# HeadReaper-hc/PL-inertial-slam

Measured on AMD Instinct MI355X. Metric: local-BA iterations/sec (50 KF, 20k pts, 4k lines, IMU), higher is better.
Workload: dtype f64; 1 GPU; configs[2]: 50 KF / 20k points / 4k lines + IMU preintegration edges (9-DoF PVR + 6-DoF bias vertices); K=50, points=20000, lines=4000, point_obs=86023, line_obs=17197, pose_dim=735, dense_dim=357, banded_twisted_solve=False, twin_factorisation=True, fused_landmark_passes=True

## Files before the change

### include/plba.h

```cpp
#ifndef PLBA_H
#define PLBA_H

#include <stddef.h>
#include <stdint.h>

#ifdef __cplusplus
extern "C" {
#endif

typedef struct plba_problem plba_problem;

typedef enum {
    PLBA_OK = 0,
    PLBA_ERR_INVALID = -1,
    PLBA_ERR_STATE = -2,
    PLBA_ERR_DEVICE = -3,
    PLBA_ERR_NUMERIC = -4,
    PLBA_ERR_EXCHANGE = -5
} plba_status;

typedef enum {
    PLBA_EDGE_POINT = 0,
    PLBA_EDGE_LINE = 1,
    PLBA_EDGE_IMU_PVR = 2,
// ... 12 lines not shown
    int    device;
    int    use_mfma;
    int    profile;
    int    factor_block;
    int    factor_flow;
    int    chain_elim;
    int    wide_steps;
    int    band_solve;
    int    marg_exact;
    int    lm_fused;
    int    lm_fused_min_obs;
    int    lm_group_steps;
    int    chain_seg;
    int    twin_max_tiles;
    int    diag;
    int    pgo_solver;
} plba_options;
#define PLBA_DIAG_TIMING 1
#define PLBA_DIAG_MARG_DUMP 2
#define PLBA_DIAG_LEAD_WAIT_FAIL 4
#define PLBA_DIAG_NO_MARG_PREROTATE 8

void plba_default_options(plba_options* o);

typedef struct {
    int    iterations;
    int    trials;
    int    stop_reason;
    int    solver_failures;
    double chi2_initial;
// ... 289 lines not shown
```

### pl-inertial-slam_amd/abi.py

```python
import ctypes as C
import numpy as np

c_double_p = C.POINTER(C.c_double)
c_int32_p = C.POINTER(C.c_int32)
c_uint8_p = C.POINTER(C.c_uint8)

EDGE_POINT, EDGE_LINE, EDGE_IMU_PVR, EDGE_IMU_BIAS, EDGE_PRIOR = range(5)

STATUS = {0: "PLBA_OK", -1: "PLBA_ERR_INVALID", -2: "PLBA_ERR_STATE", -3: "PLBA_ERR_DEVICE",
          -4: "PLBA_ERR_NUMERIC", -5: "PLBA_ERR_EXCHANGE"}


class Options(C.Structure):
    _fields_ = [("tau", C.c_double), ("good_step_lower", C.c_double), ("good_step_upper", C.c_double),
                ("max_trials", C.c_int), ("user_lambda_init", C.c_double), ("marg_eps", C.c_double),
                ("fix_line_position_jacobian", C.c_int),
                ("device", C.c_int), ("use_mfma", C.c_int), ("profile", C.c_int), ("factor_block", C.c_int), ("factor_flow", C.c_int), ("chain_elim", C.c_int), ("wide_steps", C.c_int), ("band_solve", C.c_int), ("marg_exact", C.c_int), ("lm_fused", C.c_int),
                ("lm_fused_min_obs", C.c_int), ("lm_group_steps", C.c_int), ("chain_seg", C.c_int), ("twin_max_tiles", C.c_int), ("diag", C.c_int),
                ("pgo_solver", C.c_int)]


class Stats(C.Structure):
    _fields_ = [("iterations", C.c_int), ("trials", C.c_int), ("stop_reason", C.c_int),
                ("solver_failures", C.c_int), ("chi2_initial", C.c_double), ("chi2_final", C.c_double),
                ("lambda_final", C.c_double), ("ms_total", C.c_double), ("ms_phase", C.c_double * 8)]


class TraceRow(C.Structure):
    _fields_ = [("iteration", C.c_int), ("trial", C.c_int), ("accepted", C.c_int), ("solver_ok", C.c_int),
                ("lam", C.c_double), ("chi2_current", C.c_double), ("chi2_trial", C.c_double),
                ("scale", C.c_double), ("rho", C.c_double)]


class Prior(C.Structure):
# ... 839 lines not shown
```

### pl-inertial-slam_amd/csrc/plba_api.hip

```cpp
#include <atomic>
#include <algorithm>
#include <thread>
#include <array>
#include <chrono>
#include <cmath>
#include <cstdio>
#include <cstring>
#include <condition_variable>
#include <functional>
#include <map>
#include <mutex>

#include "plba_problem.h"

using namespace plba;

namespace {
char g_create_err[256] = "";
static std::mutex g_ctx_mu;
static std::vector<HostCtx> g_ctx_free;
static std::map<int, hipStream_t> g_lib_stream;
static std::vector<plba_problem*> g_parked;
static const size_t PARK_MAX = 2;
}
// ... 45 lines not shown
    o->good_step_lower = 1. / 3.;
    o->good_step_upper = 2. / 3.;
    o->max_trials = 10;
    o->user_lambda_init = 0.0;
    o->marg_eps = 1e-8;
    o->device = -1;
    o->use_mfma = 1;
    o->factor_block = 32;
    o->factor_flow = 0;
    o->chain_elim = 1;
    o->wide_steps = 0;
    o->band_solve = 1;
    o->marg_exact = 1;
    o->lm_fused = 1;
    o->lm_fused_min_obs = 40000;
}
const char* plba_backend_name(void) { return "hip-gfx950"; }
const char* plba_last_error(const plba_problem* p) { return p ? p->err : g_create_err; }

int plba_create(const plba_options* opt, plba_problem** out) {
    if (!out) { snprintf(g_create_err, sizeof g_create_err, "out is NULL"); return PLBA_ERR_INVALID; }
    *out = nullptr;
    int ndev = 0;
    hipError_t e = hipGetDeviceCount(&ndev);
    if (e != hipSuccess || ndev == 0) {
        snprintf(g_create_err, sizeof g_create_err, "no HIP device available (%s); the plba product path has no CPU fallback",
                 e == hipSuccess ? "0 devices" : hipGetErrorString(e));
        return PLBA_ERR_DEVICE;
    }
    {
// ... 957 lines not shown
    d.imu_i = p->d_imu_i.p; d.imu_j = p->d_imu_j.p; d.imu_pre = p->d_imu_pre.p; d.imu_info_pvr = p->d_imu_ipvr.p; d.imu_info_bias = p->d_imu_ibias.p;
    d.imu_err = p->d_imu_err.p; d.imu_chi = p->d_imu_chi.p;
    d.pr_n = p->pr_n; d.pr_nv = p->pr_nv;
    d.pr_kf = p->d_pr_kf.p; d.pr_isbias = p->d_pr_isbias.p; d.pr_size = p->d_pr_size.p; d.pr_idx = p->d_pr_idx.p;
    d.pr_x0off = p->d_pr_x0off.p; d.pr_off = p->d_pr_off.p; d.pr_x0 = p->d_pr_x0.p; d.pr_J0 = p->d_pr_J0.p; d.pr_r0 = p->d_pr_r0.p;
    if (pr_dev) { d.pr_x0 = pr_dev; d.pr_J0 = pr_dev + pr_nx; d.pr_r0 = pr_dev + pr_nx + (size_t)p->pr_n * p->pr_n; }
    d.pr_err = p->d_pr_err.p; d.pr_dx = p->d_pr_dx.p; d.pr_chi = p->d_pr_chi.p;
    d.Hconst = p->d_Hconst.p; d.Himu = p->d_Himu.p; d.bimu = p->d_bimu.p; d.Himu_alt = p->d_Himu2.p; d.bimu_alt = p->d_bimu2.p; d.bprior = p->d_bprior.p; d.bprior_alt = p->d_bprior2.p; d.sys = p->d_sys.p; d.Lfac = p->d_Lfac.p; d.bpg = p->d_bpg.p; d.x = p->d_x.p;
    d.Linv = p->d_Linv.p; d.flow_flags = p->d_flow_flags.p; d.LTblk = p->d_LT32.p; d.Linv32 = p->d_LT32.p; d.rdblk = p->d_rd32.p; d.fb = (p->opt.factor_block == 64) ? 64 : 32; d.chol_flags = p->d_chol_flags.p; d.flow = p->opt.factor_flow != 0; d.wide = p->opt.wide_steps != 0 && !d.flow;
    d.chi_part = p->d_chi_part.p; d.scale_part = p->d_scale_part.p; d.maxd_part = p->d_maxd_part.p; d.kfdiag = p->d_kfdiag.p; d.posediag = p->d_posediag.p;
    d.ctrl = p->d_ctrl.p; d.trace = p->d_trace.p; d.trace_cap = TRACE_CAP; d.trace_n = p->d_trace_n.p;
    std::vector<int32_t> skey;
    {
        skey.reserve(64 + 2 * (size_t)K + 2 * (size_t)M + 4 * (size_t)p->pr_nv + ((size_t)K * K + 3) / 4 * 2 + K);
        for (int v : {K, M, p->pr_nv, p->pr_n, (int)lm_cand, p->world, p->rank, p->opt.chain_elim, p->opt.use_mfma, p->opt.factor_block, p->opt.factor_flow, p->opt.wide_steps, p->opt.band_solve,
                      p->opt.chain_seg, p->opt.twin_max_tiles, (int)(E > 300000), (int)p->lm_disable, p->P}) skey.push_back(v);
        skey.insert(skey.end(), p->off_pvr.begin(), p->off_pvr.end()); skey.insert(skey.end(), p->off_bias.begin(), p->off_bias.end());
        skey.insert(skey.end(), w.imu_i.begin(), w.imu_i.end()); skey.insert(skey.end(), w.imu_j.begin(), w.imu_j.end());
        skey.insert(skey.end(), pr_kf.begin(), pr_kf.end()); skey.insert(skey.end(), pr_isb.begin(), pr_isb.end()); skey.insert(skey.end(), p->pr_size.begin(), p->pr_size.begin() + p->pr_nv); skey.insert(skey.end(), pr_off.begin(), pr_off.end());
        skey.insert(skey.end(), p->pr_idx.begin(), p->pr_idx.begin() + p->pr_nv);
        auto pack = [&](const std::vector<uint8_t>& v) { for (size_t i = 0; i < v.size(); i += 4) { int32_t w = 0; for (size_t j = i; j < std::min(i + 4, v.size()); ++j) w |= (int32_t)(v[j] & 0xFF) << (8 * (j - i)); skey.push_back(w); } };
        pack(cov);
        if (lm_cand) { pack(LH.cov); skey.insert(skey.end(), LH.row_kf.begin(), LH.row_kf.end()); skey.push_back(LH.wmax); }
    }
    const bool sc_hit = p->sc.valid && skey == p->sc.key;
    struct BatchSwitch {
        DevBatch* prev; std::vector<std::pair<void*, size_t>>* prevlog;
        BatchSwitch(DevBatch* b, std::vector<std::pair<void*, size_t>>* log) : prev(darr_batch()), prevlog(darr_zero_log()) { darr_batch() = b; darr_zero_log() = log; }
        ~BatchSwitch() { darr_batch() = prev; darr_zero_log() = prevlog; }
    };
    if (sc_hit) {
// ... 193 lines not shown
                            }
                        for (int idx = 0; idx < n * 9; ++idx) oR[idx] = cidx[(size_t)i0 * 9 + idx] >= 0 ? cidx[(size_t)i0 * 9 + idx] : -1;
                    }
                    if ((size_t)p->Ppad * ld >= ((size_t)1 << 30)) ok = false;
                    HIPCK(p, p->d_esrc.upload(esrc));
                    cv.esrc = p->d_esrc.p; cv.esrc_off = nullptr;
                }
                p->d_W.release();
                HIPCK(p, p->d_W.alloc((size_t)(nel * 9 + 4) * cv.Wld)); HIPCK(p, p->d_Ldinv.alloc((size_t)nel * 81)); HIPCK(p, p->d_Lsub.alloc((size_t)nel * 81));
                const size_t sysn_d = (size_t)(cv.Pdpad + TILE) * cv.Pdpad;
                HIPCK(p, p->d_sysd.alloc(sysn_d)); HIPCK(p, p->d_Lfacd.alloc(sysn_d)); HIPCK(p, p->d_xd.alloc(cv.Pdpad));
                HIPCK(p, p->d_Linvd.alloc((size_t)((cv.Pdpad + TILE - 1) / TILE) * TILE * TILE)); HIPCK(p, p->d_LT32d.alloc((size_t)cv.Pdpad * 64)); HIPCK(p, p->d_rd32d.alloc(cv.Pdpad));
                HIPCK(p, p->d_flow_flagsd.alloc((cv.Pdpad + TILE - 1) / TILE)); HIPCK(p, p->d_chol_flagsd.alloc((size_t)(cv.Pdpad / 32 + 2) * (cv.Pdpad / 32)));
                cv.cidx = p->d_cidx.p; cv.epos = p->d_epos.p; cv.seg_start = p->d_seg_start.p; cv.seg_col = p->d_seg_col.p;
                cv.pidx = p->d_pidx.p; cv.ppos = p->d_ppos.p; cv.pslot = p->d_pslot.p; cv.slotcol = p->d_slotcol.p;
                cv.W = p->d_W.p; cv.Ldinv = p->d_Ldinv.p; cv.Lsub = p->d_Lsub.p;
                DevBuf& dd = p->dd;
                dd = d;
                dd.P = cv.Pd; dd.Ppad = cv.Pdpad; dd.ld = cv.Pdpad;
                dd.sys = p->d_sysd.p; dd.Lfac = p->d_Lfacd.p; dd.x = p->d_xd.p; dd.Linv = p->d_Linvd.p; dd.LTblk = p->d_LT32d.p; dd.Linv32 = p->d_LT32d.p;
                dd.rdblk = p->d_rd32d.p; dd.flow_flags = p->d_flow_flagsd.p; dd.chol_flags = p->d_chol_flagsd.p;
                dd.Ninv = nullptr; dd.Nwork = nullptr;
                if (cv.Pdpad / 32 <= NINV_MAX_T) { HIPCK(p, p->d_Ninvd.alloc((size_t)2 * cv.Pdpad * cv.Pdpad)); dd.Ninv = p->d_Ninvd.p; dd.Nwork = dd.Ninv + (size_t)cv.Pdpad * cv.Pdpad; }
                p->chain_ok = true;
            }
        }
    }
    lap("chain maps + buffers");
    d.Ninv = nullptr; d.Nwork = nullptr;
    HIPCK(p, p->d_dbgbuf.alloc(128)); d.dbgbuf = p->d_dbgbuf.p; p->dd.dbgbuf = d.dbgbuf;
    if (!p->chain_ok && p->P > 0 && p->Ppad / 32 <= NINV_MAX_T) { HIPCK(p, p->d_Ninv.alloc((size_t)2 * p->Ppad * p->ld)); d.Ninv = p->d_Ninv.p; d.Nwork = d.Ninv + (size_t)p->Ppad * p->ld; }
// ... 167 lines not shown
        }
        for (int r = 0; r < p->Ppad; ++r) xl.push_back(r * ld + r);
        std::sort(xl.begin(), xl.end());
        xl.erase(std::unique(xl.begin(), xl.end()), xl.end());
        HIPCK(p, p->d_xlist.upload(xl));
        d.xlist = p->d_xlist.p; d.nxlist = (int)xl.size();
    }
    p->band_ok = false; p->twin_ok = false;
    for (double& v : p->plan_twin) v = 0.0;
    p->dd.band = 0; p->dd.twin_m0 = 0; p->dd.twin_fac = nullptr; p->dd.cs_order = nullptr; p->dd.perm = nullptr; p->dd.xmap = nullptr; p->dd.alt = nullptr; p->dd.alt2 = nullptr;
    p->dd.wtw = nullptr;
    if (p->chain_ok && p->lm_ok && p->world <= 1) {
        const int T = p->cv.Pdpad / 32;
        HIPCK(p, p->d_wtw.alloc((size_t)(T * (T + 1) / 2 + T) * 1024, false));
        p->dd.wtw = p->d_wtw.p;
    }
    int plan_hbt = -1;
    if (p->chain_ok && p->opt.band_solve && !p->dv.flow && !p->dv.wide) {
        const ChainView& cv = p->cv;
        const int T = cv.Pdpad / 32;
        int hbt = 0;
        if (T >= 8) {
            const std::vector<int32_t>& hpidx = p->h_pidx; const std::vector<int32_t>& hsegcol = p->h_seg_col;
            std::vector<int32_t> dense_of(p->ld, -1);
            for (int c = 0; c < cv.Pd; ++c) dense_of[hpidx[c]] = c;
            for (int32_t idx : p->h_alist) {
                const int r = dense_of[idx / p->ld], c = dense_of[idx % p->ld];
                if (r >= 0 && c >= 0) hbt = std::max(hbt, std::abs(r / 32 - c / 32));
            }
            for (int g = 0; g < cv.nseg; ++g) if (hsegcol[2 * g + 1] > hsegcol[2 * g]) hbt = std::max(hbt, (hsegcol[2 * g + 1] - 1) / 32 - hsegcol[2 * g] / 32);
// ... 992 lines not shown
        std::vector<double> h; HIPCK(p, fetch(d.erec, ((size_t)p->win.Ep + 2 * (size_t)p->win.El) * EREC_UNIT, h));
        if (w == "err_pt") { v.resize((size_t)p->win.Ep * 2); for (int e = 0; e < p->win.Ep; ++e) { const size_t o = (size_t)p->ob_pos[e] * EREC_UNIT; v[2 * (size_t)e] = h[o + EREC_PT_E0]; v[2 * (size_t)e + 1] = h[o + EREC_PT_E0 + 1]; } }
        else { v.assign((size_t)p->win.El * 3, 0.0); for (int e = 0; e < p->win.El; ++e) { const size_t o = (size_t)p->ob_pos[p->win.Ep + e] * EREC_UNIT; v[3 * (size_t)e] = h[o + 13]; v[3 * (size_t)e + 1] = h[o + 14]; } }
    } else if (w == "erec") {
        if (p->lm_ok) FAIL(p, PLBA_ERR_STATE, "\"erec\": the fused landmark passes keep no record table");
        HIPCK(p, fetch(d.erec, ((size_t)p->win.Ep + 2 * (size_t)p->win.El) * EREC_UNIT, v));
    }
    else if (w == "stamps") { HIPCK(p, fetch(d.maxd_part, 80, v)); }
    else if (w == "dbgbuf") { HIPCK(p, fetch(d.dbgbuf, 128, v)); }
    else if (w == "pose_dim") v = {(double)p->P};
    else if (w == "marg_path") v.assign(p->marg_path, p->marg_path + 5);
    else if (w == "prof_lin_launches") v = {(double)p->prof_lin_launches};
    else if (w == "lm_groups") v = p->lm_hist;
    else if (w == "lm_fused") v = {(double)(p->lm_ok ? 1 : 0), (double)p->lv.ngrp, (double)p->lv.nblk, p->lm_ok && p->lm_hist.size() > 18 ? p->lm_hist[18] : 0.0 };
    else if (w == "marg_J") v = p->marg_dbg;
    else if (w == "dense_dim") v = {(double)(p->chain_ok ? p->cv.Pd : p->P)};
    else if (w == "band") v = {(double)(p->band_ok ? 1 : 0)};
    else if (w == "twin") v = {(double)(p->twin_ok ? 1 : 0)};
    else if (w == "solver_plan") {
        const bool ninv = !p->band_ok && (p->chain_ok ? p->dd.Ninv : p->dv.Ninv) != nullptr;
        v = {(double)(p->band_ok ? 3 : p->twin_ok ? 2 : p->chain_ok ? 1 : 0), (double)((p->chain_ok ? p->cv.Pdpad : p->Ppad) / 32), ninv ? 1.0 : 0.0, (double)p->plan_hbt,
             p->plan_twin[0], p->plan_twin[1], p->plan_twin[2], p->plan_twin[3], p->plan_twin[4], (double)(p->band_ok ? p->bandv.nA : 0), (double)(p->band_ok ? p->bandv.nB : 0)};
    }
    else if (w == "fact_launches_estimate") v = {(double)p->seg_launch_est};
    else if (w == "fact_launches") {
        if (p->band_ok) v = {2.0};
        else if (p->twin_ok) v = {(double)(p->twinv.nlaunch + (p->twinv.T - p->twinv.final0 - 1))};
        else v = {-1.0};
    }
    else if (w == "chi2") { HIPCK(p, plba_d2h(p, p->h_ctrl, d.ctrl, sizeof(Ctrl))); v = {p->h_ctrl->current_chi}; }
// ... 10 lines not shown
```

### pl-inertial-slam_amd/csrc/plba_chain.hip

```cpp
#include "plba_internal.h"
#include "plba_chain_dev.h"
#include "plba_factor32_dev.h"

namespace plba {

__global__ __launch_bounds__(ELIM_THREADS) void k_chain_elim(DevBuf d, ChainView cv) {
    __shared__ __attribute__((aligned(16))) ChainElimLds LDS;
    chain_elim_segment(d, cv, blockIdx.x, LDS);
}

template <bool PRE>
__global__ __launch_bounds__(256) void k_chain_schur(DevBuf d, ChainView cv, DevBuf dd) {
    __shared__ __attribute__((aligned(16))) double sC0[32 * LS];
    __shared__ __attribute__((aligned(16))) Look32 S0;
    const int T = cv.Pdpad / 32;
    const int b = blockIdx.x;
    int ta, tb;
    chain_schur_tile_of(cv, dd, b, ta, tb);
    const int wv = threadIdx.x >> 6, lane = threadIdx.x & 63, li = lane & 15, lk = lane >> 4;
    const int tr = wv >> 1, tc = wv & 1;
    const int ldd = dd.ld;
    const bool rhs_row = (ta == T);
    double4v acc;
    if (PRE) acc = *reinterpret_cast<const double4v*>(dd.wtw + (size_t)b * 1024 + 4 * threadIdx.x);
    double aold[4];
    {
        const int cb = tb * 32 + tc * 16 + li;
        const int pb = cb < cv.Pd ? cv.pidx[cb] : 0;
#pragma unroll
        for (int v = 0; v < 4; ++v) {
            const int lr = tr * 16 + lk + 4 * v;
// ... 30 lines not shown
            if (fsel >= 0) sC0[(frev ? 31 - lr : lr) * LS + (frev ? 31 - lc : lc)] = out;
        }
    }
    if (fsel < 0 || dd.flow || dd.wide || dd.band) return;
    factor32_reset(S0, threadIdx.x);
    __syncthreads();
    factor32_tile<false>(dd, fsel & 0xffff, sC0, S0, wv, lane);
}

void launch_chain_elim(const DevBuf& d, const ChainView& cv, hipStream_t s) {
    hipLaunchKernelGGL(k_chain_elim, dim3(cv.nseg), dim3(ELIM_THREADS), 0, s, d, cv);
}
bool chain_schur_factors_tile0(const DevBuf& dd) { return !dd.flow && !dd.wide && !dd.band; }
void launch_chain_schur(const DevBuf& d, const ChainView& cv, const DevBuf& dd, hipStream_t s, bool products_done) {
    const int T = cv.Pdpad / 32;
    if (products_done) hipLaunchKernelGGL(k_chain_schur<true>, dim3(T * (T + 1) / 2 + T), dim3(256), 0, s, d, cv, dd);
    else hipLaunchKernelGGL(k_chain_schur<false>, dim3(T * (T + 1) / 2 + T), dim3(256), 0, s, d, cv, dd);
}

}
```

### pl-inertial-slam_amd/csrc/plba_chain_dev.h

```cpp
#pragma once
#include "plba_internal.h"

namespace plba {

typedef double double4v __attribute__((ext_vector_type(4)));

namespace chain_detail {
__device__ __forceinline__ double lane_bcast(double v, int l) {
    int lo = __double2loint(v), hi = __double2hiint(v);
    lo = __builtin_amdgcn_readlane(lo, l);
    hi = __builtin_amdgcn_readlane(hi, l);
    return __hiloint2double(hi, lo);
}
__device__ __forceinline__ double rsqrt_full(double d) {
    double y = __builtin_amdgcn_rsq(d);
    y = y * fma(-0.5 * d * y, y, 1.5);
    y = y * fma(-0.5 * d * y, y, 1.5);
    return y;
}
template <typename T> __device__ __forceinline__ void lds_store(T* p, T v) { __hip_atomic_store(p, v, __ATOMIC_RELAXED, __HIP_MEMORY_SCOPE_WORKGROUP); }
template <typename T> __device__ __forceinline__ T lds_load(const T* p) { return __hip_atomic_load(const_cast<T*>(p), __ATOMIC_RELAXED, __HIP_MEMORY_SCOPE_WORKGROUP); }
__device__ __forceinline__ double sym_at(const double* sys, int ld, int i, int j) { return i >= j ? sys[(size_t)i * ld + j] : sys[(size_t)j * ld + i]; }
constexpr int SPIN_MAX = 1 << 20;
constexpr int SEGMAX = CHAIN_SEG;
// ... 222 lines not shown
#pragma unroll
            for (int u = 0; u < 8; ++u) {
                const int r = s0 + 32 * ch + 4 * u + lk;
                const bool in = r < rhi;
                av[ch][u] = in ? Wa[(size_t)r * cv.Wld] : 0.0;
                bv[ch][u] = in ? Wb[(size_t)r * cv.Wld] : 0.0;
            }
#pragma unroll
        for (int ch = 0; ch < NCH; ++ch)
#pragma unroll
            for (int u = 0; u < 8; ++u) acc = __builtin_amdgcn_mfma_f64_16x16x4f64(av[ch][u], bv[ch][u], acc, 0, 0, 0);
    }
    return acc;
}

}
```

### pl-inertial-slam_amd/csrc/plba_internal.h

```cpp
#pragma once
#include <hip/hip_runtime.h>
#include <stdint.h>
#include <map>
#include <mutex>
#include <string>
#include <utility>
#include <vector>

#include "plba.h"
#include "plba_math.h"
#include "plba_twin_plan.h"

namespace plba {

constexpr int TILE = 64;

inline hipError_t ensure_dyn_lds(const void* func, int bytes) {
    static std::mutex mu;
    static std::map<std::pair<int, const void*>, int> done;
    int dev = 0;
    hipError_t e = hipGetDevice(&dev);
    if (e != hipSuccess) return e;
    std::lock_guard<std::mutex> lk(mu);
    auto it = done.find({dev, func});
// ... 173 lines not shown
    const int32_t* ppos;
    const int32_t* pslot;
    const int32_t* slotcol;
    const int32_t* trow;
    const int32_t* kfpos;
    const int32_t* ekf;
    const int32_t* ukf;
    int nukf;
    const int32_t* esrc;
    const int32_t* esrc_off;
    const int32_t* bkf;
    const int32_t* imu_loc;
    double* W;
    double* Ldinv;
    double* Lsub;
};
constexpr int BAND_HB = 3;
constexpr int TWIN_MAX_TILES = 64;
constexpr int BAND_MIN_TILES = 24;
struct BandView {
    int T, nA, nB;
    double* Lband;
    double* y;
    double* mid;
};
size_t band_lds_bytes(int Pdpad);
void launch_band_solve(const DevBuf& dd, const BandView& bv, hipStream_t s);
void launch_chain_elim(const DevBuf& d, const ChainView& cv, hipStream_t s);
void launch_chain_schur(const DevBuf& d, const ChainView& cv, const DevBuf& dd, hipStream_t s, bool products_done = false);
struct TwinView {
// ... 28 lines not shown
```

### pl-inertial-slam_amd/csrc/plba_kernels.hip

```cpp
#include "plba_internal.h"
#include "plba_chain_dev.h"

namespace plba {

#define DEV __device__ __forceinline__

DEV double wave_sum(double v) {
#pragma unroll
    for (int o = 32; o > 0; o >>= 1) v += __shfl_down(v, o, 64);
    return v;
}
DEV double wave_max(double v) {
#pragma unroll
    for (int o = 32; o > 0; o >>= 1) v = fmax(v, __shfl_down(v, o, 64));
    return v;
}
DEV double block_sum_256(double v, double* s4) {
    v = wave_sum(v);
    int w = threadIdx.x >> 6;
    if ((threadIdx.x & 63) == 0) s4[w] = v;
    __syncthreads();
    double r = 0;
    if (threadIdx.x == 0) r = (s4[0] + s4[1]) + (s4[2] + s4[3]);
    __syncthreads();
// ... 677 lines not shown
    const bool ok = d.ctrl->solver_ok != 0;
    if (ok && has_pvr) kf_oplus_pvr(s, u9, tmp);
    if (ok && has_bias) {
#pragma unroll
        for (int i = 0; i < 6; ++i) tmp[16 + i] = s[16 + i] + ub6[i];
    }
}
DEV void update_kf_vals(const DevBuf& d, int trial, int k, const double* s , const double* u9, const double* ub6, bool has_pvr, bool has_bias) {
    double tmp[KF_STRIDE];
    kf_trial_state(d, s, u9, ub6, has_pvr, has_bias, tmp);
    double* o = d.kf[trial] + (size_t)k * KF_STRIDE;
#pragma unroll
    for (int i = 0; i < KF_STRIDE; ++i) publish(o + i, tmp[i]);
}

template <bool LOCAL = false>
DEV const double* chain_back_segment(const DevBuf& d, const ChainView& cv, const double* xd, const int g, const int cur, const int trial) {
    constexpr int BACK_THREADS = LMB;
    constexpr int UFAST = 5;
    __shared__ double sv[SEGMAX * 9];
    __shared__ double sxc[SEGMAX * 9];
    __shared__ double sxw[192];
    __shared__ double sM[SEGMAX][162];
#ifdef PLBA_STAMPS_LM
    unsigned long long cts[6]; cts[0] = __builtin_readcyclecounter();
#define CSTAMP(i) cts[i] = __builtin_readcyclecounter()
#else
#define CSTAMP(i) do {} while (0)
#endif
    const int wv = threadIdx.x >> 6, lane = threadIdx.x & 63, t = threadIdx.x;
    const int i0 = cv.seg_start[g], n = cv.seg_start[g + 1] - i0;
    const int wlo = cv.seg_col[2 * g], wn = cv.seg_col[2 * g + 1] - wlo;
    const int lg = t >> 4, ll = t & 15;
    constexpr int NPASS = (SEGMAX * 9 + 15) / 16;
    double wr[NPASS][UFAST], wbv[NPASS];
#pragma unroll
    for (int q = 0; q < NPASS; ++q) {
        const int r = q * 16 + lg;
        const bool in = r < n * 9;
        const double* Wr = cv.W + (size_t)(i0 * 9 + (in ? r : 0)) * cv.Wld + wlo;
#pragma unroll
        for (int u = 0; u < UFAST; ++u) { const int c = ll + 16 * u; wr[q][u] = Wr[c < wn ? c : 0]; }
        wbv[q] = Wr[cv.Pd - wlo];
    }
    int kf_k = -1, e_blk = -1;
    const int32_t* kd = nullptr;
    if (LOCAL) {}
    else if (t < n) { e_blk = t; kd = cv.bkf + (size_t)(g * CHAIN_SEG + t) * 20; }
    else if (g == 0 && t >= 64 && t - 64 < cv.nukf && t - 64 < BACK_THREADS - 64) kd = cv.bkf + (size_t)(cv.nseg * CHAIN_SEG + (t - 64)) * 20;
    double ks[KF_STRIDE];
    int op = -1, ob = -1, pc[6] = {-1, -1, -1, -1, -1, -1}, cc[9] = {-1, -1, -1, -1, -1, -1, -1, -1, -1};
    if (kd) {
        const int4* k4 = reinterpret_cast<const int4*>(kd);
        const int4 a0 = k4[0], a1 = k4[1], a2 = k4[2], a3 = k4[3], a4 = k4[4];
        kf_k = a0.x; op = a0.y; ob = a0.z;
        pc[0] = a0.w; pc[1] = a1.x; pc[2] = a1.y; pc[3] = a1.z; pc[4] = a1.w; pc[5] = a2.x;
        cc[0] = a2.y; cc[1] = a2.z; cc[2] = a2.w; cc[3] = a3.x; cc[4] = a3.y; cc[5] = a3.z; cc[6] = a3.w; cc[7] = a4.x; cc[8] = a4.y;
        const double* sp = d.kf[cur] + (size_t)kf_k * KF_STRIDE;
#pragma unroll
        for (int i = 0; i < KF_STRIDE; ++i) ks[i] = sp[i];
    }
    for (int idx = t; idx < n * 81; idx += BACK_THREADS) {
        sM[idx / 81][idx % 81] = cv.Ldinv[(size_t)i0 * 81 + idx];
        sM[idx / 81][81 + idx % 81] = cv.Lsub[(size_t)i0 * 81 + idx];
    }
    if (!LOCAL && g == 0) for (int c = t; c < cv.Pd; c += BACK_THREADS) publish(&d.x[cv.pidx[c]], xd[c]);
    for (int c = t; c < wn; c += BACK_THREADS) sxw[c] = xd[wlo + c];
    double u9[9] = {0, 0, 0, 0, 0, 0, 0, 0, 0}, ub6[6] = {0, 0, 0, 0, 0, 0};
    if (kf_k >= 0) {
        const int ps[6] = {0, 1, 2, 6, 7, 8};
#pragma unroll
        for (int i = 0; i < 6; ++i) if (pc[i] >= 0) u9[ps[i]] = xd[pc[i]];
#pragma unroll
        for (int i = 0; i < 3; ++i) if (cc[i] >= 0) u9[3 + i] = xd[cc[i]];
#pragma unroll
        for (int i = 0; i < 6; ++i) if (cc[3 + i] >= 0) ub6[i] = xd[cc[3 + i]];
    }
    __syncthreads();
    CSTAMP(1);
#pragma unroll
    for (int q = 0; q < NPASS; ++q) {
        const int r = q * 16 + lg;
        double sacc = 0.0;
#pragma unroll
        for (int u = 0; u < UFAST; ++u) { const int c = ll + 16 * u; sacc = fma(wr[q][u], c < wn ? sxw[c] : 0.0, sacc); }
        if (wn > 16 * UFAST && r < n * 9) {
            const double* Wr = cv.W + (size_t)(i0 * 9 + r) * cv.Wld + wlo;
            for (int c = 16 * UFAST + ll; c < wn; c += 16) sacc = fma(Wr[c], sxw[c], sacc);
        }
        sacc += dpp_get<0x111, 0xf>(sacc);
        sacc += dpp_get<0x112, 0xf>(sacc);
        sacc += dpp_get<0x114, 0xf>(sacc);
        sacc += dpp_get<0x118, 0xf>(sacc);
        if (ll == 15 && r < n * 9) sv[r] = wbv[q] - sacc;
    }
    __syncthreads();
    CSTAMP(2);
    if (wv == 0) {
        const int r = lane < 9 ? lane : 8;
        double xn = 0.0;
        for (int i = n - 1; i >= 0; --i) {
            const double* Li = sM[i];
            const double* Ls = Li + 81;
            double tt = sv[i * 9 + r];
            if (i + 1 < n) {
#pragma unroll
                for (int q = 0; q < 9; ++q) tt = fma(-Ls[q * 9 + r], lane_bcast(xn, q), tt);
            }
            double xi = 0.0;
#pragma unroll
            for (int q = 0; q < 9; ++q) xi = fma(Li[q * 9 + r], lane_bcast(tt, q), xi);
            xn = xi;
            const int gi = cv.cidx[(i0 + i) * 9 + r];
            if (lane < 9) { sxc[i * 9 + r] = gi >= 0 ? xi : 0.0; if (!LOCAL && gi >= 0) publish(&d.x[gi], xi); }
        }
    }
    __syncthreads();
    CSTAMP(3);
    if (LOCAL) return sxc;
    if (kf_k >= 0) {
        if (e_blk >= 0) {
#pragma unroll
            for (int i = 0; i < 3; ++i) u9[3 + i] = sxc[e_blk * 9 + i];
#pragma unroll
            for (int i = 0; i < 6; ++i) ub6[i] = sxc[e_blk * 9 + 3 + i];
            if (op >= 0) { publish(&d.x[op], u9[0]); publish(&d.x[op + 1], u9[1]); publish(&d.x[op + 2], u9[2]); publish(&d.x[op + 6], u9[6]); publish(&d.x[op + 7], u9[7]); publish(&d.x[op + 8], u9[8]); }
        }
        update_kf_vals(d, trial, kf_k, ks, u9, ub6, op >= 0, ob >= 0);
    }
    if (g == 0) for (int u = BACK_THREADS - 64 + t; u < cv.nukf; u += BACK_THREADS) update_kf_one(d, cur, trial, cv.ukf[u]);
#ifdef PLBA_STAMPS_LM
    asm volatile("s_waitcnt vmcnt(0)" ::: "memory");
    CSTAMP(4);
    if (threadIdx.x == 0 && g < 2) { for (int q = 0; q < 5; ++q) d.dbgbuf[48 + 6 * g + q] = (double)(cts[q] - cts[0]); d.dbgbuf[48 + 6 * g + 5] = (double)(long long)__builtin_amdgcn_s_memrealtime(); }
// ... 101 lines not shown
    __shared__ double sKF[2 * KF_STRIDE];
    __shared__ double sJ[9 * 24];
    __shared__ double sOJ[9 * 24];
    __shared__ double sE[16];
    __shared__ double sT[16];
    __shared__ double sW[2];
    __shared__ int sOff[24];
    const int ki = d.imu_i[m], kj = d.imu_j[m];
    const double* si = d.kf[state] + (size_t)ki * KF_STRIDE;
    const double* sj = d.kf[state] + (size_t)kj * KF_STRIDE;
    if (loc && loc->cv->imu_loc) {
        const ChainView& cvl = *loc->cv;
        const int32_t* il = cvl.imu_loc + 4 * (size_t)m;
        const int seg = il[0];
        const double* sxc = nullptr;
        if (seg >= 0) sxc = chain_back_segment<true>(d, cvl, loc->xd, seg, loc->cur, state);
        if (lane < 2) {
            const int k = lane ? kj : ki, dsc = il[1 + lane];
            const double* s = d.kf[loc->cur] + (size_t)k * KF_STRIDE;
            double ks[KF_STRIDE], u9[9] = {0, 0, 0, 0, 0, 0, 0, 0, 0}, ub6[6] = {0, 0, 0, 0, 0, 0}, tmp[KF_STRIDE];
#pragma unroll
            for (int i = 0; i < KF_STRIDE; ++i) ks[i] = s[i];
            bool has_pvr = false, has_bias = false;
            if (dsc >= 0) {
                const int32_t* kd = cvl.bkf + (size_t)dsc * 20;
                has_pvr = kd[1] >= 0; has_bias = kd[2] >= 0;
                const int ps[6] = {0, 1, 2, 6, 7, 8};
#pragma unroll
                for (int i = 0; i < 6; ++i) if (kd[3 + i] >= 0) u9[ps[i]] = loc->xd[kd[3 + i]];
                const int e = dsc - seg * CHAIN_SEG;
                if (seg >= 0 && e >= 0 && e < CHAIN_SEG && dsc < cvl.nseg * CHAIN_SEG) {
// ... 472 lines not shown
}
template <bool JAC, bool WIDE_OK>
__global__ __launch_bounds__(LMB) void k_lm_trial(DevBuf d, LmView lv, int cur, int trial, Robust rb, ChainView cv, const double* xd, int nlead, int npose, unsigned back_target, DecideArgs da) {
    static_assert(LMB == 256, "chain_back_segment's thread layout");
    __shared__ double s4[4];
    int b = blockIdx.x;
    const int nimu_first = (nlead > 0 && npose > 0 && cv.imu_loc && gridDim.x <= 512) ? min(npose, d.M) : 0;
    if (b >= nlead && b < nlead + nimu_first) {
        const LocalStates loc{&cv, xd, cur};
        pose_edge_block<JAC, 256>(d, trial, rb, b - nlead, threadIdx.x, nullptr, 0, s4, nullptr, &loc);
        if (da.fuse) trial_arrive(d, da, lv.ngrp, s4);
        return;
    }
    if (b >= nlead + nimu_first) b -= nimu_first;
    if (b < nlead) {
        chain_back_segment(d, cv, xd, b, cur, trial);
        lead_done(d.back_cnt);
    } else if (b < nlead + lv.ngrp) {
        __shared__ LmLds S;
        const int g = b - nlead;
        if (g == 0 && nlead == 0) {
            for (int k = threadIdx.x; k < d.K; k += LMB) update_kf_one(d, cur, trial, k);
            lead_done(d.back_cnt);
        }
        const int kind = lv.grp[g].kind;
        if (kind == 0) lm_trial_group<false, false>(d, lv, g, cur, trial, rb, cv, xd, nlead != 0, S);
        else if (kind == 1) lm_trial_group<true, false>(d, lv, g, cur, trial, rb, cv, xd, nlead != 0, S);
        else if (WIDE_OK && kind == 2) lm_trial_group<false, true>(d, lv, g, cur, trial, rb, cv, xd, nlead != 0, S);
        else if (WIDE_OK) lm_trial_group<true, true>(d, lv, g, cur, trial, rb, cv, xd, nlead != 0, S);
    } else {
        const int m = b - nlead - lv.ngrp + nimu_first;
// ... 246 lines not shown
```

### pl-inertial-slam_amd/csrc/plba_problem.h

```cpp
#pragma once
#include <algorithm>
#include <chrono>
#include <cstring>
#include <map>
#include <mutex>
#include <utility>
#include <vector>

#include "plba_internal.h"
#include "plba_window.h"

namespace plba {

struct DevPool {
    static constexpr size_t POOL_CAP = (size_t)8 << 30;
    std::mutex mu;
    std::map<std::pair<int, size_t>, std::vector<void*>> free_;
    size_t cached = 0;
    size_t n_malloc = 0, n_reuse = 0;
    static size_t size_class(size_t bytes) { size_t c = 4096; while (c < bytes) c <<= 1; return c; }
    hipError_t get(size_t bytes, void** out, size_t* cls) {
        int dev = 0;
        (void)hipGetDevice(&dev);
        *cls = size_class(bytes);
// ... 199 lines not shown
    plba::DArr<char> d_batch_z, d_batch_u;
    plba::DevBatch batch;
    struct StructCache {
        bool valid = false;
        std::vector<int32_t> key;
        plba::DevBuf dd;
        const int32_t *alist = nullptr, *xlist = nullptr, *alist2 = nullptr; int nalist = 0, nxlist = 0, nalist2 = 0;
        const uint8_t* col_gather = nullptr;
        double *Ninv = nullptr, *Nwork = nullptr, *dbgbuf = nullptr;
        bool chain_ok = false;
        std::vector<std::pair<void*, size_t>> zero_log;
        long hits = 0, misses = 0;
    } sc;
    plba::DArr<char> d_sbatch_z, d_sbatch_u;
    plba::DevBatch sbatch;
    plba::DArr<double> d_wtw;
    plba::DArr<double> d_twin_alt;
    plba::Window win, win_next;
    plba::SlidePlan slide;
    int pr_n = 0, pr_nv = 0;
    std::vector<int32_t> pr_vid, pr_size, pr_idx;
    std::vector<double> pr_x0, pr_J0, pr_r0;
    plba::DArr<double> d_prd[2];
    int prd_slot = 0;
    bool prior_dev = false;
    bool prior_changed = false;
    int pr_m = 0;
    plba::MargPending* mp = nullptr;
    double pgo_sparse[8] = {0, 0, 0, 0, 0, 0, 0, 0};
    long host_waits = 0;
// ... 135 lines not shown
```

Baseline: 7812 iterations/s.

## Precompute chain back-substitution map so per-trial back-solve becomes a matvec

Adds a precomputed per-segment map G, built once in extra blocks of the chain Schur kernel, that folds the block-bidiagonal back-substitution into the W coupling matrix. The per-trial chain_back_segment then reads G instead of W, skips loading Ldinv/Lsub and the serial 9x9 triangular sweep, and publishes x directly. This moves the sequential dependency chain out of the per-LM-trial critical path and into the once-per-iteration factorization. The cost is an extra G buffer and additional work in the Schur kernel. It is enabled by default through a new option.

```diff
diff --git a/include/plba.h b/include/plba.h
--- a/include/plba.h
+++ b/include/plba.h
@@ -50,6 +50,7 @@
     int    chain_seg;
     int    twin_max_tiles;
     int    diag;
+    int    chain_back_map;
     int    pgo_solver;
 } plba_options;
 #define PLBA_DIAG_TIMING 1
diff --git a/pl-inertial-slam_amd/abi.py b/pl-inertial-slam_amd/abi.py
--- a/pl-inertial-slam_amd/abi.py
+++ b/pl-inertial-slam_amd/abi.py
@@ -17,7 +17,7 @@
                 ("fix_line_position_jacobian", C.c_int),
                 ("device", C.c_int), ("use_mfma", C.c_int), ("profile", C.c_int), ("factor_block", C.c_int), ("factor_flow", C.c_int), ("chain_elim", C.c_int), ("wide_steps", C.c_int), ("band_solve", C.c_int), ("marg_exact", C.c_int), ("lm_fused", C.c_int),
                 ("lm_fused_min_obs", C.c_int), ("lm_group_steps", C.c_int), ("chain_seg", C.c_int), ("twin_max_tiles", C.c_int), ("diag", C.c_int),
-                ("pgo_solver", C.c_int)]
+                ("chain_back_map", C.c_int), ("pgo_solver", C.c_int)]
 
 
 class Stats(C.Structure):
diff --git a/pl-inertial-slam_amd/csrc/plba_api.hip b/pl-inertial-slam_amd/csrc/plba_api.hip
--- a/pl-inertial-slam_amd/csrc/plba_api.hip
+++ b/pl-inertial-slam_amd/csrc/plba_api.hip
@@ -83,6 +83,7 @@
     o->marg_exact = 1;
     o->lm_fused = 1;
     o->lm_fused_min_obs = 40000;
+    o->chain_back_map = 1;
 }
 const char* plba_backend_name(void) { return "hip-gfx950"; }
 const char* plba_last_error(const plba_problem* p) { return p ? p->err : g_create_err; }
@@ -1070,7 +1071,7 @@
     {
         skey.reserve(64 + 2 * (size_t)K + 2 * (size_t)M + 4 * (size_t)p->pr_nv + ((size_t)K * K + 3) / 4 * 2 + K);
         for (int v : {K, M, p->pr_nv, p->pr_n, (int)lm_cand, p->world, p->rank, p->opt.chain_elim, p->opt.use_mfma, p->opt.factor_block, p->opt.factor_flow, p->opt.wide_steps, p->opt.band_solve,
-                      p->opt.chain_seg, p->opt.twin_max_tiles, (int)(E > 300000), (int)p->lm_disable, p->P}) skey.push_back(v);
+                      p->opt.chain_seg, p->opt.chain_back_map, p->opt.twin_max_tiles, (int)(E > 300000), (int)p->lm_disable, p->P}) skey.push_back(v);
         skey.insert(skey.end(), p->off_pvr.begin(), p->off_pvr.end()); skey.insert(skey.end(), p->off_bias.begin(), p->off_bias.end());
         skey.insert(skey.end(), w.imu_i.begin(), w.imu_i.end()); skey.insert(skey.end(), w.imu_j.begin(), w.imu_j.end());
         skey.insert(skey.end(), pr_kf.begin(), pr_kf.end()); skey.insert(skey.end(), pr_isb.begin(), pr_isb.end()); skey.insert(skey.end(), p->pr_size.begin(), p->pr_size.begin() + p->pr_nv); skey.insert(skey.end(), pr_off.begin(), pr_off.end());
@@ -1294,7 +1295,7 @@
                 HIPCK(p, p->d_flow_flagsd.alloc((cv.Pdpad + TILE - 1) / TILE)); HIPCK(p, p->d_chol_flagsd.alloc((size_t)(cv.Pdpad / 32 + 2) * (cv.Pdpad / 32)));
                 cv.cidx = p->d_cidx.p; cv.epos = p->d_epos.p; cv.seg_start = p->d_seg_start.p; cv.seg_col = p->d_seg_col.p;
                 cv.pidx = p->d_pidx.p; cv.ppos = p->d_ppos.p; cv.pslot = p->d_pslot.p; cv.slotcol = p->d_slotcol.p;
-                cv.W = p->d_W.p; cv.Ldinv = p->d_Ldinv.p; cv.Lsub = p->d_Lsub.p;
+                cv.W = p->d_W.p; cv.Ldinv = p->d_Ldinv.p; cv.Lsub = p->d_Lsub.p; cv.G = nullptr;
                 DevBuf& dd = p->dd;
                 dd = d;
                 dd.P = cv.Pd; dd.Ppad = cv.Pdpad; dd.ld = cv.Pdpad;
@@ -1492,6 +1493,10 @@
         const int T = p->cv.Pdpad / 32;
         HIPCK(p, p->d_wtw.alloc((size_t)(T * (T + 1) / 2 + T) * 1024, false));
         p->dd.wtw = p->d_wtw.p;
+        if (p->opt.chain_back_map) {
+            HIPCK(p, p->d_G.alloc((size_t)(p->cv.nel * 9 + 4) * p->cv.Wld, false));
+            p->cv.G = p->d_G.p;
+        }
     }
     int plan_hbt = -1;
     if (p->chain_ok && p->opt.band_solve && !p->dv.flow && !p->dv.wide) {
@@ -2514,6 +2519,7 @@
     else if (w == "lm_groups") v = p->lm_hist;
     else if (w == "lm_fused") v = {(double)(p->lm_ok ? 1 : 0), (double)p->lv.ngrp, (double)p->lv.nblk, p->lm_ok && p->lm_hist.size() > 18 ? p->lm_hist[18] : 0.0 };
     else if (w == "marg_J") v = p->marg_dbg;
+    else if (w == "chain_back_map") v = {(double)(p->opt.chain_back_map ? 1 : 0), (double)((p->chain_ok && p->cv.G) ? 1 : 0)};
     else if (w == "dense_dim") v = {(double)(p->chain_ok ? p->cv.Pd : p->P)};
     else if (w == "band") v = {(double)(p->band_ok ? 1 : 0)};
     else if (w == "twin") v = {(double)(p->twin_ok ? 1 : 0)};
diff --git a/pl-inertial-slam_amd/csrc/plba_chain.hip b/pl-inertial-slam_amd/csrc/plba_chain.hip
--- a/pl-inertial-slam_amd/csrc/plba_chain.hip
+++ b/pl-inertial-slam_amd/csrc/plba_chain.hip
@@ -15,6 +15,11 @@
     __shared__ __attribute__((aligned(16))) Look32 S0;
     const int T = cv.Pdpad / 32;
     const int b = blockIdx.x;
+    if (PRE && b >= T * (T + 1) / 2 + T) {
+        __shared__ ChainMapLds sMap;
+        chain_back_map_segment(cv, b - (T * (T + 1) / 2 + T), sMap);
+        return;
+    }
     int ta, tb;
     chain_schur_tile_of(cv, dd, b, ta, tb);
     const int wv = threadIdx.x >> 6, lane = threadIdx.x & 63, li = lane & 15, lk = lane >> 4;
@@ -75,7 +80,7 @@
 bool chain_schur_factors_tile0(const DevBuf& dd) { return !dd.flow && !dd.wide && !dd.band; }
 void launch_chain_schur(const DevBuf& d, const ChainView& cv, const DevBuf& dd, hipStream_t s, bool products_done) {
     const int T = cv.Pdpad / 32;
-    if (products_done) hipLaunchKernelGGL(k_chain_schur<true>, dim3(T * (T + 1) / 2 + T), dim3(256), 0, s, d, cv, dd);
+    if (products_done) hipLaunchKernelGGL(k_chain_schur<true>, dim3(T * (T + 1) / 2 + T + (cv.G ? cv.nseg : 0)), dim3(256), 0, s, d, cv, dd);
     else hipLaunchKernelGGL(k_chain_schur<false>, dim3(T * (T + 1) / 2 + T), dim3(256), 0, s, d, cv, dd);
 }
 
diff --git a/pl-inertial-slam_amd/csrc/plba_chain_dev.h b/pl-inertial-slam_amd/csrc/plba_chain_dev.h
--- a/pl-inertial-slam_amd/csrc/plba_chain_dev.h
+++ b/pl-inertial-slam_amd/csrc/plba_chain_dev.h
@@ -260,4 +260,65 @@
     return acc;
 }
 
-}
+struct ChainMapLds {
+    alignas(16) double sM[SEGMAX][162];
+    int live[SEGMAX * 9];
+};
+__device__ __forceinline__ void chain_back_map_segment(const ChainView& cv, const int g, ChainMapLds& S) {
+    const int i0 = cv.seg_start[g], n = cv.seg_start[g + 1] - i0;
+    const int wlo = cv.seg_col[2 * g], wn = cv.seg_col[2 * g + 1] - wlo;
+    if (n <= 0) return;
+    const int lc = threadIdx.x;
+    const bool act = lc <= wn;
+    const int col = lc == wn ? cv.Pd : wlo + (act ? lc : 0);
+    constexpr int AHEAD = 3;
+    double w[SEGMAX][9];
+    auto request = [&](int j) {
+        const double* Wc = cv.W + (size_t)((i0 + (j < n ? n - 1 - j : 0)) * 9) * cv.Wld + col;
+#pragma unroll
+        for (int r = 0; r < 9; ++r) w[j][r] = Wc[(size_t)r * cv.Wld];
+    };
+#pragma unroll
+    for (int j = 0; j < AHEAD; ++j) request(j);
+    for (int idx = threadIdx.x; idx < n * 81; idx += blockDim.x) {
+        S.sM[idx / 81][idx % 81] = cv.Ldinv[(size_t)i0 * 81 + idx];
+        S.sM[idx / 81][81 + idx % 81] = cv.Lsub[(size_t)i0 * 81 + idx];
+    }
+    for (int idx = threadIdx.x; idx < n * 9; idx += blockDim.x) S.live[idx] = cv.cidx[(size_t)i0 * 9 + idx] >= 0;
+    __syncthreads();
+    if ((int)(threadIdx.x & ~63u) > wn) return;
+    double gn[9];
+#pragma unroll
+    for (int r = 0; r < 9; ++r) gn[r] = 0.0;
+#pragma unroll
+    for (int j = 0; j < SEGMAX; ++j) {
+        if (j >= n) break;
+        if (j + AHEAD < SEGMAX) request(j + AHEAD);
+        const int i = n - 1 - j;
+        const double* Li = S.sM[i];
+        const double* Ls = Li + 81;
+        double t[9];
+#pragma unroll
+        for (int r = 0; r < 9; ++r) t[r] = w[j][r];
+        if (j > 0) {
+#pragma unroll
+            for (int q = 0; q < 9; ++q)
+#pragma unroll
+                for (int r = 0; r < 9; ++r) t[r] = fma(-Ls[q * 9 + r], gn[q], t[r]);
+        }
+#pragma unroll
+        for (int r = 0; r < 9; ++r) {
+            double x = 0.0;
+#pragma unroll
+            for (int q = r; q < 9; ++q) x = fma(Li[q * 9 + r], t[q], x);
+            gn[r] = x;
+        }
+        if (act) {
+            double* Gc = cv.G + (size_t)((i0 + i) * 9) * cv.Wld + col;
+#pragma unroll
+            for (int r = 0; r < 9; ++r) Gc[(size_t)r * cv.Wld] = S.live[i * 9 + r] ? gn[r] : 0.0;
+        }
+    }
+}
+
+}
diff --git a/pl-inertial-slam_amd/csrc/plba_internal.h b/pl-inertial-slam_amd/csrc/plba_internal.h
--- a/pl-inertial-slam_amd/csrc/plba_internal.h
+++ b/pl-inertial-slam_amd/csrc/plba_internal.h
@@ -211,6 +211,7 @@
     double* W;
     double* Ldinv;
     double* Lsub;
+    double* G;
 };
 constexpr int BAND_HB = 3;
 constexpr int TWIN_MAX_TILES = 64;
diff --git a/pl-inertial-slam_amd/csrc/plba_kernels.hip b/pl-inertial-slam_amd/csrc/plba_kernels.hip
--- a/pl-inertial-slam_amd/csrc/plba_kernels.hip
+++ b/pl-inertial-slam_amd/csrc/plba_kernels.hip
@@ -715,14 +715,19 @@
     for (int i = 0; i < KF_STRIDE; ++i) publish(o + i, tmp[i]);
 }
 
-template <bool LOCAL = false>
+struct ChainBackLds {
+    double sv[SEGMAX * 9];
+    double sxc[SEGMAX * 9];
+    double sxw[192];
+    double sM[SEGMAX][162];
+};
+DEV ChainBackLds& chain_back_lds() { __shared__ ChainBackLds s; return s; }
+template <bool LOCAL = false, bool MAP = false>
 DEV const double* chain_back_segment(const DevBuf& d, const ChainView& cv, const double* xd, const int g, const int cur, const int trial) {
     constexpr int BACK_THREADS = LMB;
     constexpr int UFAST = 5;
-    __shared__ double sv[SEGMAX * 9];
-    __shared__ double sxc[SEGMAX * 9];
-    __shared__ double sxw[192];
-    __shared__ double sM[SEGMAX][162];
+    ChainBackLds& S = chain_back_lds();
+    auto& sv = S.sv; auto& sxc = S.sxc; auto& sxw = S.sxw; auto& sM = S.sM;
 #ifdef PLBA_STAMPS_LM
     unsigned long long cts[6]; cts[0] = __builtin_readcyclecounter();
 #define CSTAMP(i) cts[i] = __builtin_readcyclecounter()
@@ -734,16 +739,18 @@
     const int wlo = cv.seg_col[2 * g], wn = cv.seg_col[2 * g + 1] - wlo;
     const int lg = t >> 4, ll = t & 15;
     constexpr int NPASS = (SEGMAX * 9 + 15) / 16;
+    const double* const Wsrc = MAP ? cv.G : cv.W;
     double wr[NPASS][UFAST], wbv[NPASS];
 #pragma unroll
     for (int q = 0; q < NPASS; ++q) {
         const int r = q * 16 + lg;
         const bool in = r < n * 9;
-        const double* Wr = cv.W + (size_t)(i0 * 9 + (in ? r : 0)) * cv.Wld + wlo;
+        const double* Wr = Wsrc + (size_t)(i0 * 9 + (in ? r : 0)) * cv.Wld + wlo;
 #pragma unroll
         for (int u = 0; u < UFAST; ++u) { const int c = ll + 16 * u; wr[q][u] = Wr[c < wn ? c : 0]; }
         wbv[q] = Wr[cv.Pd - wlo];
     }
+    const int gi_t = (MAP && !LOCAL && t < n * 9) ? cv.cidx[(size_t)i0 * 9 + t] : -1;
     int kf_k = -1, e_blk = -1;
     const int32_t* kd = nullptr;
     if (LOCAL) {}
@@ -761,7 +768,7 @@
 #pragma unroll
         for (int i = 0; i < KF_STRIDE; ++i) ks[i] = sp[i];
     }
-    for (int idx = t; idx < n * 81; idx += BACK_THREADS) {
+    if (!MAP) for (int idx = t; idx < n * 81; idx += BACK_THREADS) {
         sM[idx / 81][idx % 81] = cv.Ldinv[(size_t)i0 * 81 + idx];
         sM[idx / 81][81 + idx % 81] = cv.Lsub[(size_t)i0 * 81 + idx];
     }
@@ -786,18 +793,22 @@
 #pragma unroll
         for (int u = 0; u < UFAST; ++u) { const int c = ll + 16 * u; sacc = fma(wr[q][u], c < wn ? sxw[c] : 0.0, sacc); }
         if (wn > 16 * UFAST && r < n * 9) {
-            const double* Wr = cv.W + (size_t)(i0 * 9 + r) * cv.Wld + wlo;
+            const double* Wr = Wsrc + (size_t)(i0 * 9 + r) * cv.Wld + wlo;
             for (int c = 16 * UFAST + ll; c < wn; c += 16) sacc = fma(Wr[c], sxw[c], sacc);
         }
         sacc += dpp_get<0x111, 0xf>(sacc);
         sacc += dpp_get<0x112, 0xf>(sacc);
         sacc += dpp_get<0x114, 0xf>(sacc);
         sacc += dpp_get<0x118, 0xf>(sacc);
-        if (ll == 15 && r < n * 9) sv[r] = wbv[q] - sacc;
-    }
-    __syncthreads();
+        if (ll == 15 && r < n * 9) {
+            const double vr = wbv[q] - sacc;
+            if (MAP) sxc[r] = vr;
+            else sv[r] = vr;
+        }
+    }
+    if (!MAP) __syncthreads();
     CSTAMP(2);
-    if (wv == 0) {
+    if (!MAP && wv == 0) {
         const int r = lane < 9 ? lane : 8;
         double xn = 0.0;
         for (int i = n - 1; i >= 0; --i) {
@@ -819,6 +830,7 @@
     __syncthreads();
     CSTAMP(3);
     if (LOCAL) return sxc;
+    if (MAP && gi_t >= 0) publish(&d.x[gi_t], sxc[t]);
     if (kf_k >= 0) {
         if (e_blk >= 0) {
 #pragma unroll
@@ -950,7 +962,8 @@
         const int32_t* il = cvl.imu_loc + 4 * (size_t)m;
         const int seg = il[0];
         const double* sxc = nullptr;
-        if (seg >= 0) sxc = chain_back_segment<true>(d, cvl, loc->xd, seg, loc->cur, state);
+        if (seg >= 0) sxc = cvl.G ? chain_back_segment<true, true>(d, cvl, loc->xd, seg, loc->cur, state)
+                                  : chain_back_segment<true, false>(d, cvl, loc->xd, seg, loc->cur, state);
         if (lane < 2) {
             const int k = lane ? kj : ki, dsc = il[1 + lane];
             const double* s = d.kf[loc->cur] + (size_t)k * KF_STRIDE;
@@ -1453,7 +1466,8 @@
     }
     if (b >= nlead + nimu_first) b -= nimu_first;
     if (b < nlead) {
-        chain_back_segment(d, cv, xd, b, cur, trial);
+        if (cv.G) chain_back_segment<false, true>(d, cv, xd, b, cur, trial);
+        else chain_back_segment<false, false>(d, cv, xd, b, cur, trial);
         lead_done(d.back_cnt);
     } else if (b < nlead + lv.ngrp) {
         __shared__ LmLds S;
diff --git a/pl-inertial-slam_amd/csrc/plba_problem.h b/pl-inertial-slam_amd/csrc/plba_problem.h
--- a/pl-inertial-slam_amd/csrc/plba_problem.h
+++ b/pl-inertial-slam_amd/csrc/plba_problem.h
@@ -237,6 +237,7 @@
     } sc;
     plba::DArr<char> d_sbatch_z, d_sbatch_u;
     plba::DevBatch sbatch;
+    plba::DArr<double> d_G;
     plba::DArr<double> d_wtw;
     plba::DArr<double> d_twin_alt;
     plba::Window win, win_next;
```

Result: slower. 7684 iterations/s (-1.6%).
